# jalhajj/mahout

Measured on AMD Instinct MI355X. Metric: sketch updates/sec + item-pair cosines/sec @1M items, 1/2/4/8 MI355X, higher is better.
Workload: dtype u32

## Files before the change

mahout_amd/csrc/cms_build.hip:

```cpp
#include <hip/hip_runtime.h>

#include <algorithm>
#include <cstdlib>

#include "cms_device.h"
#include "cms_internal.h"

namespace cms {

#ifdef CMS_BUILD_CHEAPHASH
#define bucket(hp, d, kp) ((uint32_t)(((kp) >> (d)) & (hp).wmask))
#endif
#ifdef CMS_BUILD_GATHERHASH
#define bucket(hp, d, kp) \
  ((uint32_t)(((&(hp).gtab[(kp) & 0xFFFFFFu].x)[((d) >> 1) & 3] >> (((d) & 1) << 4)) & (hp).wmask))
#endif

struct HotInfo {
  int64_t row;
  int32_t nslices;
  int32_t e0;
};

constexpr int kKeyRegs = 4;

typedef unsigned short u16x2 __attribute__((ext_vector_type(2)));

__device__ __forceinline__ uint32_t nibbles8(uint32_t lo, uint32_t hi) {
  return __builtin_amdgcn_perm(hi | (hi >> 4), lo | (lo >> 4), 0x06040200u);
}

__global__ void k_build_plan(const int64_t* lo_, const int64_t* hi_, int64_t nrows, int64_t split, int64_t slice,
                             int first, int32_t* row_hot, HotInfo* hot, int2* extra_map,
                             uint32_t* counters , uint64_t* norm, uint32_t* rowmax,
                             int depth) {
  const int lane = (int)__lane_id();
  for (int64_t base = blockIdx.x * (int64_t)blockDim.x; base < nrows; base += (int64_t)gridDim.x * blockDim.x) {
    const int64_t r = base + threadIdx.x;
    const int64_t c = r < nrows ? hi_[r] - lo_[r] : 0;
    const bool is_hot = c > split;
    if (r < nrows && !is_hot) row_hot[r] = -1;
    int32_t ns = 0;
    uint32_t hidx = 0, e0 = 0;
    if (is_hot) {
      ns = (int32_t)((c + slice - 1) / slice);
      const unsigned long long old =
          atomicAdd(reinterpret_cast<unsigned long long*>(counters), ((unsigned long long)(ns - first) << 32) | 1ULL);
      hidx = (uint32_t)old;
      e0 = (uint32_t)(old >> 32);
      hot[hidx] = HotInfo{r, ns, (int32_t)e0};
      row_hot[r] = (int32_t)hidx;
      for (int d = 0; d < depth; ++d) norm[r * depth + d] = 0;
      rowmax[r] = 0;
    }
    unsigned long long m = __ballot(is_hot);
    while (m) {
      const int l = __builtin_ctzll(m);
      m &= m - 1;
      const int32_t nsl = __builtin_amdgcn_readlane(ns, l);
      const uint32_t hl = (uint32_t)__builtin_amdgcn_readlane((int)hidx, l);
      const uint32_t el = (uint32_t)__builtin_amdgcn_readlane((int)e0, l);
      for (int32_t sl = first + lane; sl < nsl; sl += 64) extra_map[el + sl - first] = make_int2((int)hl, sl);
    }
  }
}

__global__ void k_row_bound_implicit(const int64_t* lo_, const int64_t* hi_, int64_t nrows, int fb, int64_t slice, const uint64_t* old_mass,
                                     uint64_t* bound, uint8_t* force) {
  for (int64_t r = blockIdx.x * (int64_t)blockDim.x + threadIdx.x; r < nrows; r += (int64_t)gridDim.x * blockDim.x) {
    const int64_t c = hi_[r] - lo_[r];
    bound[r] = ((uint64_t)c << fb) + (old_mass ? old_mass[r] : 0ULL);
    force[r] = c > slice ? 1 : 0;
  }
}

__global__ __launch_bounds__(256) void k_row_bound_values(const int64_t* lo_, const int64_t* hi_, const float* vals, int64_t nrows, int fb,
                                                          int64_t slice, const uint64_t* old_mass, uint64_t* bound,
                                                          uint8_t* force) {
  __shared__ uint64_t red[4];
  for (int64_t r = blockIdx.x; r < nrows; r += gridDim.x) {
    uint64_t s = 0;
    for (int64_t i = lo_[r] + threadIdx.x; i < hi_[r]; i += 256) {
      uint32_t inc;
      if (load_inc(vals, i, inc, fb)) s += inc;
    }
    s = block_sum_u64_sat(s, red);
    if (threadIdx.x == 0) {
      bound[r] = sat_add(s, old_mass ? old_mass[r] : 0ULL);
      force[r] = (hi_[r] - lo_[r]) > slice ? 1 : 0;
    }
  }
}

constexpr int64_t kByteKeys = 64 * kKeyRegs;
__device__ __forceinline__ bool byte_class(int32_t slot, int64_t nkeys, uint64_t bound) {
  return slot < 0 && nkeys <= kByteKeys && bound < 256;
}

typedef uint32_t u32x4_t __attribute__((ext_vector_type(4)));
__device__ __forceinline__ void store_row(uint4* p, uint4 v, int sv) {
  if (sv == 2) {
    const u32x4_t x = {v.x, v.y, v.z, v.w};
    __builtin_nontemporal_store(x, reinterpret_cast<u32x4_t*>(p));
  } else {
    *p = v;
  }
}

#ifdef CMS_NO_SLICE_PAIRS
constexpr bool kNoSlicePairs = true;
#else
constexpr bool kNoSlicePairs = false;
#endif
constexpr int kBuildStoreForm = 2;
constexpr size_t kFormLdsMax = 64 * 1024;

constexpr int kBuildWaves = 6;
template <int SV>
__global__ __launch_bounds__(kBuildThreads) __attribute__((amdgpu_waves_per_eu(kBuildWaves, 8))) void k_build_rows(
    const int64_t* lo_, const int64_t* hi_, Keys keys, const float* vals, int64_t nrows, HashParams hp,
    int64_t slice,
    const int32_t* row_hot, const HotInfo* hot, const int2* extra_map, const uint32_t* counters, int64_t emax,
    TableView tv, uint64_t* row_mass, uint64_t* norm, uint32_t* rowmax, uint32_t* flags, int accumulate,
    int slices_done, const uint64_t* bound, int forms, int skip_untouched, int32_t* hidx_w, uint32_t* cbound,
    const int32_t* rows_list, const uint32_t* rows_cnt) {
  extern __shared__ __align__(16) uint32_t lds[];
  __shared__ unsigned long long s_norm[CMS_MAX_DEPTH];
  __shared__ unsigned long long s_mass;
  __shared__ uint32_t s_max;
  const int w = (int)hp.width;
  const int64_t dw = (int64_t)hp.depth * w;
  const int tid = threadIdx.x;

  int64_t row, lo, hi;
  bool atomic_mode;
  if (blockIdx.x < emax) {
    if (slices_done || blockIdx.x >= counters[1]) return;
#ifdef CMS_BUILD_NOSLICES
    return;
#endif
    int2 m = extra_map[blockIdx.x];
    row = hot[m.x].row;
    lo = lo_[row] + (int64_t)m.y * slice;
    hi = min(hi_[row], lo + slice);
    atomic_mode = true;
  } else {
    row = (int64_t)blockIdx.x - emax;
    if (rows_list) {
      if (row >= (int64_t)*rows_cnt) return;
      row = rows_list[row];
    }
    lo = lo_[row];
    atomic_mode = row_hot[row] >= 0;
    if (atomic_mode && slices_done) return;
    hi = atomic_mode ? lo + slice : hi_[row];
    if (skip_untouched && hi_[row] == lo) return;
// ... 472 lines not shown
            const int64_t i = base + tid + (int64_t)u * MTH;
            inc4[u] = 0;
            if (i < hi) {
              uint32_t inc;
              if (!load_inc(vals, i, inc, hp.frac_bits)) {
                badv = true;
                inc = 0;
              }
              inc4[u] = inc;
            }
          }
          if (base + kStep < hi) fetch(base + kStep);
#pragma unroll
          for (int u = 0; u < 4; ++u) {
            if (inc4[u]) add_all(keys.resolve(kk[u]), inc4[u], -1);
            mass += inc4[u];
          }
        }
        mass_pending = false;
      }
      if (__ballot(ovf) && (tid & 63) == 0) s_ovf = 1u;
      __syncthreads();
      const bool fits = s_ovf == 0u;
      __syncthreads();
      if (fits) level = 0;
      if (fits && tele) {
#pragma unroll
        for (int d = 0; d < kSq; ++d) {
          const uint32_t sq = wave_sum_u32(sqr[d]);
          if ((tid & 63) == 0 && sq) atomicAdd(&s_norm[d], (unsigned long long)sq);
        }
        level = 3;
      }
    }
    if (level == 3) level = 0;
    else if (level == 0) {
      const uint4* l4 = reinterpret_cast<const uint4*>(lds);
      const int nq = w >> 5;
      for (int d = 0; d < hp.depth; ++d) {
        uint32_t sq = 0;
        for (int j = tid; j < nq; j += MTH) {
          const uint4 v = l4[d * nq + j];
          const uint32_t x[4] = {v.x, v.y, v.z, v.w};
#pragma unroll
          for (int q = 0; q < 4; ++q) {
            const uint32_t lo4 = x[q] & 0x0F0F0F0Fu, hi4 = (x[q] >> 4) & 0x0F0F0F0Fu;
            sq = __builtin_amdgcn_udot4(lo4, lo4, sq, false);
            sq = __builtin_amdgcn_udot4(hi4, hi4, sq, false);
          }
#ifdef CMS_BUILD_NOWRITE
          if (false)
#endif
          if (!as_list) store_row(d4 + d * nq + j, v, SV);
        }
        sq = wave_sum_u32(sq);
        if ((tid & 63) == 0 && sq) atomicAdd(&s_norm[d], (unsigned long long)sq);
      }
    }
    if (level < 0) level = start > 1 ? 2 : 1;
    else level = -level - 1;
    for (;;) {
      if (level < 0) break;
      const int bits = 4 << level;
      const int lg = 3 - level;
      const uint32_t cap = (1u << bits) - 1u;
      const int nq = (w * bits) >> 7;
      uint4* l4 = reinterpret_cast<uint4*>(lds);
      if (tid < CMS_MAX_DEPTH) s_norm[tid] = 0ULL;
      if (tid == 0) {
        s_max = 0u;
        s_ovf = 0u;
        s_mass = 0ULL;
      }
      vmax = 0;
      for (int d = 0; d < hp.depth; ++d) {
        for (int j = tid; j < nq; j += MTH) l4[j] = make_uint4(0, 0, 0, 0);
        __syncthreads();
        uint64_t sq = 0;
        bool ovf = false;
        auto add = [&](uint64_t kr, uint32_t inc) {
          const uint32_t c = bucket(hp, d, kr);
          const uint32_t sh = (c & ((1u << lg) - 1u)) * (uint32_t)bits;
          const uint32_t old = (atomicAdd(&lds[c >> lg], inc << sh) >> sh) & cap;
          const uint32_t nv = old + inc;
          ovf |= nv > cap || inc > cap;
          sq += (uint64_t)(2u * old + inc) * inc;
          vmax = max(vmax, nv);
        };
        if (cached) {
#pragma unroll
          for (int k = 0; k < MKR; ++k)
            if (ik[k]) add(kp[k], ik[k]);
        } else {
          for (int64_t base = lo; base < hi; base += kMidRowKeys * MTH) {
            uint64_t kk[kMidRowKeys];
            uint32_t inc4[kMidRowKeys];
#pragma unroll
            for (int u = 0; u < kMidRowKeys; ++u) {
              const int64_t i = base + tid + (int64_t)u * MTH;
              kk[u] = i < hi ? keys.at(i) : 0;
              inc4[u] = 0;
              if (i < hi) {
                uint32_t inc;
                if (!load_inc(vals, i, inc, hp.frac_bits)) {
                  badv = true;
                  inc = 0;
                }
                inc4[u] = inc;
              }
            }
#pragma unroll
            for (int u = 0; u < kMidRowKeys; ++u) {
              if (inc4[u]) add(kk[u], inc4[u]);
              if (mass_pending) mass += inc4[u];
            }
          }
          mass_pending = false;
        }
        sq = wave_sum_u64_sat(sq);
        if ((tid & 63) == 0 && sq) atomicAdd(&s_norm[d], (unsigned long long)sq);
        if (__ballot(ovf) && (tid & 63) == 0) s_ovf = 1u;
        __syncthreads();
        if (s_ovf) break;
#ifdef CMS_BUILD_NOWRITE
        if (false)
#endif
        if (!(as_list && level == 1))
          for (int j = tid; j < nq; j += MTH) store_row(d4 + d * nq + j, l4[j], SV);
        __syncthreads();
      }
      if (!s_ovf || level == 2) break;
      __syncthreads();
      ++level;
    }
    if (level < 0) level = -level - 1;
    if (badv) atomicOr(flags, kFlagBadValue);
#pragma unroll
    for (int o = 32; o > 0; o >>= 1) vmax = max(vmax, (uint32_t)__shfl_xor((int)vmax, o, 64));
    if ((tid & 63) == 0 && vmax) atomicMax(&s_max, vmax);
    mass = wave_sum_u64_sat(mass);
    if ((tid & 63) == 0 && mass) atomicAdd(&s_mass, (unsigned long long)mass);
    __syncthreads();
    if (tid < hp.depth) norm[row * hp.depth + tid] = s_norm[tid];
    const bool listed = as_list && level <= 1;
    if (tid == 0) {
      rowmax[row] = s_max;
      row_mass[row] = s_mass;
      if (s_mass >= (1ULL << 32)) atomicOr(flags, kFlagOverflow);
      if (listed) lst[0] = (uint16_t)m;
      hidx_w[row] = listed ? kFormList : level == 0 ? kFormU4 : level == 1 ? kFormU8 : kFormU16;
      cbound[row] = s_max;
    }
    __syncthreads();
  }
}

constexpr int kStreamThreads = 512;
constexpr int kStreamPer = 2;
constexpr int kStreamRedWords = 1 + (kStreamThreads / 64) * (CMS_MAX_DEPTH + 2);
template <int SV, int D>
__device__ __forceinline__ void mid_streamed(const int64_t* lo_, const int64_t* hi_, const Keys& keys,
                                             const HashParams& hp, const int32_t* list, const uint32_t* list_cnt,
                                             uint32_t cap, const TableView& tv, int32_t* hidx_w, uint32_t* cbound,
                                             uint64_t* row_mass, uint64_t* norm, uint32_t* rowmax, int32_t* redo,
                                             uint32_t* redo_cnt, uint32_t* ticket, int u4_keys, int u8_keys) {
  extern __shared__ __align__(16) uint32_t lds[];
  constexpr int T = kStreamThreads;
  constexpr int NW = T / 64;
  constexpr int RS = CMS_MAX_DEPTH + 2;
  const int tid = threadIdx.x, lane = tid & 63, wv = tid >> 6;
  const int w = (int)hp.width;
  const int depth = D > 0 ? D : hp.depth;
  const int nq = w >> 4;
  const uint32_t nfront = list_cnt[0], count = nfront + list_cnt[1];
  uint4* l4 = reinterpret_cast<uint4*>(lds);
  uint32_t* red = lds + 1;
  if (tid == 0) lds[0] = atomicAdd(ticket, 1u);
  __syncthreads();
  uint32_t li = lds[0];
  while (li < count) {
    __syncthreads();
    const int64_t row = list2_at(list, cap, nfront, li);
    const int64_t lo = lo_[row], hi = hi_[row];
    const int64_t m = hi - lo;
    const bool u8_start = m > u4_keys && m <= u8_keys;
    uint32_t mine = 0;
    uint32_t bytes = 0;
    u16x2 pm = {0, 0};
    if (u8_start) {
      for (int j = tid; j < depth * nq; j += T) l4[j] = make_uint4(0, 0, 0, 0);
      __syncthreads();
      constexpr int64_t kStep = (int64_t)kStreamPer * T;
      uint64_t nx[kStreamPer];
      auto fetch = [&](int64_t base) {
#pragma unroll
        for (int u = 0; u < kStreamPer; ++u) {
          const int64_t i = base + tid + (int64_t)u * T;
          nx[u] = i < hi ? keys.raw(i) : 0ULL;
        }
      };
      fetch(lo);
      for (int64_t base = lo; base < hi; base += kStep) {
        uint64_t kk[kStreamPer];
#pragma unroll
        for (int u = 0; u < kStreamPer; ++u) kk[u] = nx[u];
        if (base + kStep < hi) fetch(base + kStep);
#pragma unroll
        for (int u = 0; u < kStreamPer; ++u) {
          if (base + tid + (int64_t)u * T >= hi) continue;
          each_bucket<D>(hp, keys.resolve(kk[u]), [&](int r, uint32_t bk) {
            const uint32_t c = (uint32_t)r * (uint32_t)w + bk;
            atomicAdd(&lds[c >> 2], 1u << ((c & 3u) << 3));
          });
        }
      }
      __syncthreads();
      uint4* d4 = reinterpret_cast<uint4*>(tv.row16(row));
      auto sweep_row = [&](int r) {
        uint32_t sq = 0;
        for (int j = tid; j < nq; j += T) {
          const uint4 v = l4[r * nq + j];
          const uint32_t x[4] = {v.x, v.y, v.z, v.w};
#pragma unroll
          for (int q = 0; q < 4; ++q) {
            sq = __builtin_amdgcn_udot4(x[q], x[q], sq, false);
            bytes = __builtin_amdgcn_udot4(x[q], 0x01010101u, bytes, false);
            pm = __builtin_elementwise_max(pm, __builtin_elementwise_max(__builtin_bit_cast(u16x2, x[q] & 0x00FF00FFu),
                                                                         __builtin_bit_cast(u16x2, (x[q] >> 8) & 0x00FF00FFu)));
          }
          store_row(d4 + r * nq + j, v, SV);
        }
        sq = wave_sum_u32(sq);
        if (lane == r) mine = sq;
      };
#pragma unroll 1
      for (int r = 0; r < depth; ++r) sweep_row(r);
    }
    uint32_t vmax = max((uint32_t)pm.x, (uint32_t)pm.y);
#pragma unroll
    for (int o = 32; o > 0; o >>= 1) vmax = max(vmax, (uint32_t)__shfl_xor((int)vmax, o, 64));
    bytes = wave_sum_u32(bytes);
    __syncthreads();
    if (lane < depth) red[wv * RS + lane] = mine;
    if (lane == 0) {
      red[wv * RS + CMS_MAX_DEPTH] = vmax;
      red[wv * RS + CMS_MAX_DEPTH + 1] = bytes;
    }
    if (tid == 0) lds[0] = atomicAdd(ticket, 1u);
    __syncthreads();
    uint32_t mx = 0, total = 0;
#pragma unroll
    for (int k = 0; k < NW; ++k) {
      mx = max(mx, red[k * RS + CMS_MAX_DEPTH]);
      total += red[k * RS + CMS_MAX_DEPTH + 1];
    }
    if (!u8_start || total != (uint32_t)depth * (uint32_t)m) {
      if (tid == 0) redo[atomicAdd(redo_cnt, 1u)] = (int32_t)row;
    } else {
      if (tid < depth) {
        uint64_t s = 0;
#pragma unroll
        for (int k = 0; k < NW; ++k) s += red[k * RS + tid];
        norm[row * depth + tid] = s;
      }
      if (tid == 0) {
        rowmax[row] = mx;
        row_mass[row] = (uint64_t)m;
        hidx_w[row] = kFormU8;
        cbound[row] = mx;
      }
    }
    li = lds[0];
  }
}

template <int SV, int D, int MT>
__global__ __launch_bounds__(MT) __attribute__((amdgpu_waves_per_eu(MT == kStreamThreads ? 8 : 4, 8))) void k_build_mid(
    const int64_t* lo_, const int64_t* hi_, Keys keys, const float* vals, HashParams hp,
    const int32_t* list, const uint32_t* list_cnt , uint32_t cap, TableView tv, int32_t* hidx_w,
    uint32_t* cbound, uint64_t* row_mass, uint64_t* norm, uint32_t* rowmax, uint32_t* flags, int list_keys,
    int u4_keys, int u8_keys, int32_t* redo, uint32_t* redo_cnt, uint32_t* ticket) {
  if constexpr (MT == kStreamThreads)
    mid_streamed<SV, D>(lo_, hi_, keys, hp, list, list_cnt, cap, tv, hidx_w, cbound, row_mass, norm, rowmax, redo,
                        redo_cnt, ticket, u4_keys, u8_keys);
  else
    mid_rows<SV, D, MT>(lo_, hi_, keys, vals, hp, list, list_cnt, cap, tv, hidx_w, cbound, row_mass, norm, rowmax,
                        flags, list_keys, u4_keys, u8_keys);
}

constexpr int kMidGridPerCu = 8;
constexpr int kNibWaves = 4;

__global__ void k_row_caps(const int64_t* lo_, const int64_t* hi_, int64_t n, const uint64_t* bound,
                           const int32_t* hidx, int forms, int weighted, int frac_bits, int d, int w, int bit_keys,
                           int crumb_keys, int list_keys, uint32_t* caps) {
  const int64_t dw = (int64_t)d * w;
  const uint32_t full = (uint32_t)(slot_units(dw) / kRowAlign);
  for (int64_t r = blockIdx.x * (int64_t)blockDim.x + threadIdx.x; r < n; r += (int64_t)gridDim.x * blockDim.x) {
    const int32_t s = hidx[r];
    const int64_t m = hi_[r] - lo_[r];
    uint32_t c = full;
    if (s >= 0) {
      c = 0;
    } else if (forms && byte_class(s, m, bound[r])) {
      const int64_t u16s = nib_list_row(m, w, d, weighted != 0, frac_bits, bit_keys, crumb_keys, list_keys)
                               ? 1 + (int64_t)d * m
                               : dw / 2;
      c = (uint32_t)((u16s + kRowAlign - 1) / kRowAlign);
    }
    caps[r] = c;
  }
}

template <int SV>
__device__ __forceinline__ void nib_owner(
    int64_t row, uint32_t* lds, const int64_t* lo_, const int64_t* hi_, const Keys& keys, const float* vals,
    const HashParams& hp, const int32_t* row_hot, const uint64_t* bound, const TableView& tv, int32_t* hidx_w,
    uint32_t* cbound, uint64_t* row_mass, uint64_t* norm, uint32_t* rowmax, uint32_t* flags, int32_t* redo,
    uint32_t* redo_cnt, int bit_keys, int crumb_keys, int list_keys, int lists_done) {
  const int lane = threadIdx.x & 63;
  const int wv = threadIdx.x >> 6;
  const int64_t lo = lo_[row], hi = hi_[row];
  if (row_hot[row] >= 0 || !byte_class(tv.hidx[row], hi - lo, bound[row])) return;
  const int w = (int)hp.width;
  if (lists_done && nib_list_row(hi - lo, w, hp.depth, vals != nullptr, hp.frac_bits, bit_keys, crumb_keys, list_keys))
    return;
  uint64_t kp[kKeyRegs];
  uint32_t ik[kKeyRegs];
  uint32_t mass = 0;
  bool badv = false;
#pragma unroll
  for (int k = 0; k < kKeyRegs; ++k) {
    const int64_t i = lo + lane + (int64_t)k * 64;
    kp[k] = 0;
    ik[k] = 0;
    if (i < hi) {
      uint32_t inc;
      if (!load_inc(vals, i, inc, hp.frac_bits)) {
        badv = true;
        inc = 0;
      }
      kp[k] = keys.at(i);
      ik[k] = inc;
      mass += inc;
    }
  }
  const int64_t m = hi - lo;
  int bits = nib_first_bits(m, w, bit_keys, crumb_keys);
  const bool as_list = nib_list_row(m, w, hp.depth, vals != nullptr, hp.frac_bits, bit_keys, crumb_keys, list_keys);
  if (as_list) bits = 4;
  uint16_t* lst = tv.row16(row);
  uint4* slot4 = reinterpret_cast<uint4*>(lds) + wv * (w >> 5);
  uint32_t* slot = lds + wv * (w >> 3);
  uint4* d4 = reinterpret_cast<uint4*>(tv.row16(row));
  uint32_t vmax = 0;
  bool ovf = false;
  for (;;) {
    const int lg = bits == 1 ? 5 : bits == 2 ? 4 : 3;
    const uint32_t cap = (1u << bits) - 1u;
    const int nq = (w * bits) >> 7;
    vmax = 0;
    ovf = false;
    for (int d = 0; d < hp.depth; ++d) {
      for (int j = lane; j < nq; j += 64) slot4[j] = make_uint4(0, 0, 0, 0);
      uint32_t sq = 0;
#pragma unroll
      for (int k = 0; k < kKeyRegs; ++k)
        if (ik[k]) {
// ... 376 lines not shown
#pragma unroll
    for (int r = 0; r < D; ++r) sq[r] = 0u;
    uint32_t vmax = 0;
    const int nf = min(max((m - lane + 63) >> 6, 0), NSL);
    const uint32_t live = (1u << nf) - 1u;
    const int ns = (m + 63) >> 6;
    const bool ovf = mid_list_rows<D>(slot, pk, live, ns, sq, vmax);
    if (ovf) {
      if (lane == 0) redo[atomicAdd(redo_cnt, 1u)] = row;
    } else {
#pragma unroll
      for (int r = 0; r < D; ++r) sq[r] = wave_fold_dpp(sq[r], [](uint32_t a, uint32_t b) { return a + b; });
      vmax = wave_fold_dpp(vmax, [](uint32_t a, uint32_t b) { return max(a, b); });
      if (lane < D) {
        uint32_t s = 0;
#pragma unroll
        for (int r = 0; r < D; ++r)
          if (lane == r) s = sq[r];
        norm[(int64_t)row * D + lane] = s;
      }
      if (lane == 0) {
        lst[0] = (uint16_t)m;
        rowmax[row] = vmax;
        row_mass[row] = (uint64_t)m;
        hidx_w[row] = kFormList;
        cbound[row] = vmax;
      }
    }
    if (row1 < 0) break;
    row = row1;
    lo = nlo;
    m = nm;
    base = nbase;
    raw0 = nraw0;
    row1 = row2;
  }
}

template <int SV>
__global__ __launch_bounds__(kBuildThreads) void k_build_bytes(
    const int64_t* lo_, const int64_t* hi_, Keys keys, const float* vals, HashParams hp,
    const int32_t* list, const uint32_t* list_cnt, TableView tv, int32_t* hidx_w, uint32_t* cbound,
    uint64_t* row_mass, uint64_t* norm, uint32_t* rowmax, uint32_t* flags) {
  extern __shared__ __align__(16) uint32_t lds[];
  __shared__ unsigned long long s_norm[CMS_MAX_DEPTH];
  __shared__ uint32_t s_max, s_mass;
  const int tid = threadIdx.x;
  const int w = (int)hp.width;
  const int64_t dw = (int64_t)hp.depth * w;
  const uint32_t count = *list_cnt;
  for (uint32_t li = blockIdx.x; li < count; li += gridDim.x) {
    const bool keep_list = list[li] < 0;
    const int64_t row = keep_list ? ~(int64_t)list[li] : (int64_t)list[li];
    const int64_t lo = lo_[row], hi = hi_[row];
    uint16_t* lst = tv.row16(row);
    if (tid < CMS_MAX_DEPTH) s_norm[tid] = 0ULL;
    if (tid == 0) {
      s_max = 0u;
      s_mass = 0u;
    }
    uint64_t kp[kKeyRegs];
    uint32_t ik[kKeyRegs];
    uint32_t mass = 0;
    bool badv = false;
#pragma unroll
    for (int k = 0; k < kKeyRegs; ++k) {
      const int64_t i = lo + tid + (int64_t)k * kBuildThreads;
      kp[k] = 0;
      ik[k] = 0;
      if (i < hi) {
        uint32_t inc;
        if (!load_inc(vals, i, inc, hp.frac_bits)) {
          badv = true;
          inc = 0;
        }
        kp[k] = keys.at(i);
        ik[k] = inc;
        mass += inc;
      }
    }
    const int nq = (int)(dw >> 4);
    uint4* l4 = reinterpret_cast<uint4*>(lds);
    for (int j = tid; j < nq; j += kBuildThreads) l4[j] = make_uint4(0, 0, 0, 0);
    __syncthreads();
    uint32_t vmax = 0;
    for (int d = 0; d < hp.depth; ++d) {
      uint32_t sq = 0;
#pragma unroll
      for (int k = 0; k < kKeyRegs; ++k)
        if (ik[k]) {
          const uint32_t bk = bucket(hp, d, kp[k]);
          const uint32_t c = (uint32_t)d * (uint32_t)w + bk;
          if (keep_list) lst[1 + (int64_t)d * (hi - lo) + tid + (int64_t)k * kBuildThreads] = (uint16_t)bk;
          const uint32_t sh = (c & 3u) << 3;
          const uint32_t old = (atomicAdd(&lds[c >> 2], ik[k] << sh) >> sh) & 255u;
          sq += (2u * old + ik[k]) * ik[k];
          vmax = max(vmax, old + ik[k]);
        }
      sq = wave_sum_u32(sq);
      if ((tid & 63) == 0 && sq) atomicAdd(&s_norm[d], (unsigned long long)sq);
    }
#pragma unroll
    for (int o = 32; o > 0; o >>= 1) vmax = max(vmax, (uint32_t)__shfl_xor((int)vmax, o, 64));
    if ((tid & 63) == 0 && vmax) atomicMax(&s_max, vmax);
    mass = wave_sum_u32(mass);
    if ((tid & 63) == 0 && mass) atomicAdd(&s_mass, mass);
    __syncthreads();
    uint4* d4 = reinterpret_cast<uint4*>(lst);
#ifdef CMS_BUILD_NOWRITE
    if (false)
#endif
    if (!keep_list)
      for (int j = tid; j < nq; j += kBuildThreads) store_row(d4 + j, l4[j], SV);
    if (badv) atomicOr(flags, kFlagBadValue);
    if (tid < hp.depth) norm[row * hp.depth + tid] = s_norm[tid];
    if (tid == 0) {
      rowmax[row] = s_max;
      row_mass[row] = s_mass;
      hidx_w[row] = keep_list ? kFormList : kFormU8;
      cbound[row] = s_max;
    }
    __syncthreads();
  }
}

constexpr int kSliceThreads = 512;
constexpr bool kWholeSlices = true;
constexpr int64_t kHotSlice = 65535;
template <int D>
__global__ __launch_bounds__(kSliceThreads) void k_build_slices(const int64_t* lo_, const int64_t* hi_, Keys keys,
                                                                HashParams hp, int64_t slice, const HotInfo* hot,
                                                                const int2* smap, const uint32_t* counters,
                                                                TableView tv, uint64_t* row_mass, uint32_t* flags,
                                                                int whole, uint64_t* norm, uint32_t* rowmax) {
  extern __shared__ __align__(16) uint32_t lds[];
  const uint32_t nsl = counters[1];
  if (blockIdx.x >= nsl) return;
  const int tid = threadIdx.x;
  const uint32_t stride = (nsl % 7919u) ? 7919u : 7907u;
  const uint32_t sidx = (uint32_t)(((uint64_t)blockIdx.x * stride) % nsl);
  const int2 m = smap[sidx];
  const int64_t row = hot[m.x].row;
  const int64_t lo = lo_[row] + (int64_t)m.y * slice;
  const int64_t end = min(hi_[row], lo + slice);
  const int w = (int)hp.width;
  const int64_t dw = (int64_t)hp.depth * w;
  const int words = (int)(dw >> 1);
  uint4* l4 = reinterpret_cast<uint4*>(lds);
  for (int j = tid; j < (words >> 2); j += kSliceThreads) l4[j] = make_uint4(0, 0, 0, 0);
  for (int j = (words & ~3) + tid; j < words; j += kSliceThreads) lds[j] = 0u;
  __syncthreads();
  const uint32_t one = 1u << hp.frac_bits;
  constexpr int kPer = 8;
  constexpr int64_t kStep = kPer * kSliceThreads;
  uint64_t nx[kPer];
  auto fetch = [&](int64_t base) {
#pragma unroll
    for (int u = 0; u < kPer; ++u) {
      const int64_t i = base + tid + (int64_t)u * kSliceThreads;
      nx[u] = i < end ? keys.raw(i) : 0ULL;
    }
  };
  if (lo < end) fetch(lo);
  for (int64_t base = lo; base < end; base += kStep) {
    uint64_t kk[kPer];
#pragma unroll
    for (int u = 0; u < kPer; ++u) kk[u] = nx[u];
    if (base + kStep < end) fetch(base + kStep);
#pragma unroll
    for (int u = 0; u < kPer; ++u) {
      if (base + tid + (int64_t)u * kSliceThreads >= end) continue;
      const uint64_t kp = keys.resolve(kk[u]);
      each_bucket<D>(hp, kp, [&](int r, uint32_t bk) {
        const uint32_t c = (uint32_t)r * (uint32_t)w + bk;
#ifdef CMS_BUILD_NOLDSADD
        if (c == 0xFFFFFFFFu)
#endif
        atomicAdd(&lds[c >> 1], one << ((c & 1u) << 4));
      });
    }
  }
  __syncthreads();
  if (whole && hot[m.x].nslices == 1) {
    u32x4_t* o4 = reinterpret_cast<u32x4_t*>(tv.hot + (int64_t)tv.hidx[row] * dw);
    const uint2* s2 = reinterpret_cast<const uint2*>(lds);
    uint32_t vmax = 0;
    for (int r = 0; r < hp.depth; ++r) {
      uint64_t sq = 0;
      const int q0 = r * (w >> 2), q1 = q0 + (w >> 2);
      for (int q = q0 + tid; q < q1; q += kSliceThreads) {
        const uint2 v = s2[q];
        const uint32_t c0 = v.x & 0xFFFFu, c1 = v.x >> 16, c2 = v.y & 0xFFFFu, c3 = v.y >> 16;
        sq += (uint64_t)c0 * c0 + (uint64_t)c1 * c1 + (uint64_t)c2 * c2 + (uint64_t)c3 * c3;
        vmax = max(max(vmax, max(c0, c1)), max(c2, c3));
        const u32x4_t x = {c0, c1, c2, c3};
        __builtin_nontemporal_store(x, o4 + q);
      }
      sq = wave_sum_u64_sat(sq);
      if ((tid & 63) == 0 && sq) atomicAdd((unsigned long long*)&norm[row * hp.depth + r], (unsigned long long)sq);
    }
#pragma unroll
    for (int o = 32; o > 0; o >>= 1) vmax = max(vmax, (uint32_t)__shfl_xor((int)vmax, o, 64));
    if ((tid & 63) == 0 && vmax) atomicMax(&rowmax[row], vmax);
  } else {
    unsigned long long* dst = reinterpret_cast<unsigned long long*>(tv.hot + (int64_t)tv.hidx[row] * dw);
    const int units = (words + 63) >> 6;
    const int rot = (int)(((uint32_t)m.y * 2654435761u >> 8) % (uint32_t)units) << 6;
    for (int jj = tid; jj < words; jj += kSliceThreads) {
      const int j = jj + rot < words ? jj + rot : jj + rot - words;
      const uint32_t v = lds[j];
#ifdef CMS_BUILD_NOSLICEADD
      if (v == 0xFFFFFFFFu)
#endif
      if (v) atomicAdd(dst + j, (unsigned long long)(v & 0xFFFFu) | ((unsigned long long)(v >> 16) << 32));
    }
  }
  if (tid == 0) {
    const uint64_t tm = (uint64_t)(end - lo) * one;
    const unsigned long long old = atomicAdd((unsigned long long*)&row_mass[row], (unsigned long long)tm);
    if (old + tm >= (1ULL << 32)) atomicOr(flags, kFlagOverflow);
  }
}

__global__ __launch_bounds__(256) void k_hot_norms(const HotInfo* hot, const uint32_t* counters, HashParams hp,
                                                   TableView tv, uint64_t* norm, uint32_t* rowmax, int whole_slices) {
  __shared__ uint64_t red[4];
  const uint32_t nhot = counters[0];
  const int d = blockIdx.y;
  const int w = (int)hp.width;
  for (uint32_t hb = blockIdx.x; hb < nhot; hb += gridDim.x) {
    if (hot[hb].nslices <= whole_slices) continue;
    const int64_t row = hot[hb].row;
    const uint32_t* p = tv.hot + (int64_t)tv.hidx[row] * tv.dw + (int64_t)d * w;
    uint64_t sq = 0;
    uint32_t vmax = 0;
    if ((w & 3) == 0 && (((uintptr_t)p) & 15) == 0) {
      const uint4* p4 = reinterpret_cast<const uint4*>(p);
      for (int j = threadIdx.x; j < (w >> 2); j += 256) {
        const uint4 v = p4[j];
        sq = sat_add(sq, (uint64_t)v.x * v.x + (uint64_t)v.y * v.y);
        sq = sat_add(sq, (uint64_t)v.z * v.z + (uint64_t)v.w * v.w);
        vmax = max(vmax, max(max(v.x, v.y), max(v.z, v.w)));
      }
    } else {
      for (int j = threadIdx.x; j < w; j += 256) {
        sq = sat_add(sq, (uint64_t)p[j] * p[j]);
        vmax = max(vmax, p[j]);
      }
    }
#pragma unroll
    for (int o = 32; o > 0; o >>= 1) vmax = max(vmax, (uint32_t)__shfl_xor((int)vmax, o, 64));
    if ((threadIdx.x & 63) == 0 && vmax) atomicMax(&rowmax[row], vmax);
    uint64_t tot = block_sum_u64_sat(sq, red);
    if (tot > (1ULL << 60)) tot = 1ULL << 60;
    if (threadIdx.x == 0) atomicAdd((unsigned long long*)&norm[row * hp.depth + d], (unsigned long long)tot);
  }
}

int row_bounds(cms_handle* h, const int64_t* d_lo, const int64_t* d_hi, const float* d_val, const uint64_t* old_mass,
               int64_t slice, uint64_t* bound, uint8_t* force) {
  const int64_t n = h->n;
  if (d_val)
    hipLaunchKernelGGL(k_row_bound_values, dim3((unsigned)std::max<int64_t>(1, std::min<int64_t>(n, 65536))),
                       dim3(256), 0, h->stream, d_lo, d_hi, d_val, n, h->hp.frac_bits, slice, old_mass, bound, force);
  else
    hipLaunchKernelGGL(k_row_bound_implicit, dim3((unsigned)std::max<int64_t>(1, std::min<int64_t>((n + 255) / 256, 4096))),
                       dim3(256), 0, h->stream, d_lo, d_hi, n, h->hp.frac_bits, slice, old_mass, bound, force);
  CMS_HIP(hipGetLastError());
  return CMS_OK;
}

int ingest_csr_device(cms_handle* h, const int64_t* d_off, const int64_t* d_key, const float* d_val, int64_t npairs) {
  h->rf_valid = false;
  return ingest_spans_device(h, d_off, d_off + 1, d_key, nullptr, d_val, npairs);
}

int ingest_spans_device(cms_handle* h, const int64_t* d_lo, const int64_t* d_hi, const int64_t* d_key,
                        const uint32_t* d_tok, const float* d_val, int64_t npairs) {
  const Keys keys{d_key, d_tok};
  const int64_t n = h->n;
  int rc0;
  const int accumulate = h->empty ? 0 : 1;
  int64_t kSplit = cms::kSlice;
  if (h->p.width >= 8192) kSplit *= 2;
  if (h->tune.split_keys > 0) kSplit = h->tune.split_keys;
  const size_t img_lds = (size_t)h->dw * 2;
  const bool fast_slices = !d_val && (h->dw % 8) == 0 && img_lds <= 80 * 1024 && h->hp.frac_bits < 16;
  const int64_t kSliceKeys = fast_slices ? (kHotSlice >> h->hp.frac_bits) : kSplit;
  const int whole_slices =
      kWholeSlices && fast_slices && !accumulate && (h->p.width % 4) == 0 ? 1 : 0;
  const int64_t max_hot = std::min<int64_t>(n, npairs / kSplit + 1);
  const int64_t emax = npairs / kSliceKeys + max_hot + 1;
  const size_t sz_rowhot = (sizeof(int32_t) * (size_t)n + 15) & ~size_t(15);
  const size_t sz_hot = (sizeof(HotInfo) * (size_t)max_hot + 15) & ~size_t(15);
  const size_t sz_extra = sizeof(int2) * (size_t)emax;
  CMS_HIP(h->ws_hot.ensure(sz_rowhot + sz_hot + sz_extra + 64));
  char* base = h->ws_hot.as<char>();
  int32_t* row_hot = reinterpret_cast<int32_t*>(base);
  HotInfo* hot = reinterpret_cast<HotInfo*>(base + sz_rowhot);
  int2* extra_map = reinterpret_cast<int2*>(base + sz_rowhot + sz_hot);
  uint32_t* counters = h->d_flags + 4;
  struct PlanSide {
    cms_handle* h;
    bool on = false;
    void end() {
      if (!on) return;
      on = false;
      std::swap(h->stream, h->side_stream);
      h->plan_side_active = false;
      if (hipEventRecord(h->ev_plan, h->side_stream) == hipSuccess) (void)hipStreamWaitEvent(h->stream, h->ev_plan, 0);
    }
    ~PlanSide() { end(); }
  } plan_side{h};
  if (h->spans_event && !accumulate && !d_val && h->side_stream) {
    h->spans_event = false;
    CMS_HIP(hipStreamWaitEvent(h->side_stream, h->ev_spans, 0));
    std::swap(h->stream, h->side_stream);
    h->plan_side_active = true;
    plan_side.on = true;
  }
  CMS_HIP(hipMemsetAsync(counters, 0, 4 * sizeof(uint32_t), h->stream));
  {
    TimedScope ts(h, "build_plan");
    if (!accumulate && (rc0 = reset_table_layout(h))) return rc0;
    DevBuf& bound = h->ws_bound;
    DevBuf& force = h->ws_force;
    CMS_HIP(bound.ensure(sizeof(uint64_t) * (size_t)std::max<int64_t>(n, 1)));
    CMS_HIP(force.ensure((size_t)std::max<int64_t>(n, 1)));
    if ((rc0 = row_bounds(h, d_lo, d_hi, d_val, accumulate ? h->d_row_mass : nullptr, kSplit, bound.as<uint64_t>(),
                          force.as<uint8_t>())))
      return rc0;
    int64_t max_new = -1;
    if (!accumulate && !d_val && h->hp.frac_bits < 16) {
// ... 230 lines not shown
```

mahout_amd/csrc/cms_hash.h:

```cpp
#pragma once
#include <math.h>
#include <stdint.h>

#ifndef CMS_HD
#define CMS_HD __host__ __device__ __forceinline__
#endif

#define CMS_MAX_DEPTH 32

namespace cms {

constexpr uint64_t kPrime = 9223372036854775783ULL;
constexpr uint64_t kMask63 = 0x7FFFFFFFFFFFFFFFULL;

struct HashParams {
  uint64_t ap[CMS_MAX_DEPTH];
  uint64_t bp[CMS_MAX_DEPTH];
  uint64_t barrett;
  uint32_t width;
  uint32_t wmask;
  int32_t depth;
  int32_t pow2;
  int32_t frac_bits;
  int32_t fastq;
  double qa[CMS_MAX_DEPTH];
  double qb[CMS_MAX_DEPTH];
#ifdef CMS_BUILD_GATHERHASH
  const uint4* gtab;
#endif
};

inline void hash_finish(HashParams& hp) {
  hp.pow2 = hp.width != 0 && (hp.width & (hp.width - 1)) == 0;
  hp.wmask = hp.pow2 ? hp.width - 1u : 0u;
  hp.barrett = hp.pow2 ? 0 : (~0ULL) / (uint64_t)hp.width;
  hp.fastq = hp.pow2 && hp.width <= (1u << 24);
  for (int i = 0; i < CMS_MAX_DEPTH; ++i) {
    hp.qa[i] = i < hp.depth ? (double)((long double)hp.ap[i] / (long double)kPrime) : 0.0;
    hp.qb[i] = i < hp.depth ? (double)((long double)hp.bp[i] / (long double)kPrime) : 0.0;
  }
}

CMS_HD uint64_t reduce_key(int64_t k) {
  const int64_t P = (int64_t)kPrime;
  if (k >= 0) return (uint64_t)(k >= P ? k - P : k);
  int64_t t = k + P;
  if (t < 0) t += P;
  return (uint64_t)t;
}

CMS_HD uint64_t mulmod_p(uint64_t x, uint64_t y) {
  unsigned __int128 prod = (unsigned __int128)x * y;
  uint64_t lo = (uint64_t)prod;
  uint64_t hi = (uint64_t)(prod >> 64);
  uint64_t H = (hi << 1) | (lo >> 63);
  uint64_t L = lo & kMask63;
  unsigned __int128 t = (unsigned __int128)H * 25u;
  uint64_t tH = (uint64_t)(t >> 63);
  uint64_t tL = (uint64_t)t & kMask63;
  uint64_t z = tL + L;
  if (z >= kPrime) z -= kPrime;
  if (z >= kPrime) z -= kPrime;
  z += tH * 25u;
  if (z >= kPrime) z -= kPrime;
  return z;
}

CMS_HD uint64_t mulmod_p_small(uint64_t x, uint32_t y) {
  const uint64_t p0 = (uint64_t)(uint32_t)x * y;
  const uint64_t p1 = (x >> 32) * (uint64_t)y;
  const uint64_t lo = p0 + (p1 << 32);
  const uint64_t hi = (p1 >> 32) + (lo < p0 ? 1u : 0u);
  const uint64_t H = (hi << 1) | (lo >> 63);
  uint64_t z = (lo & kMask63) + H * 25u;
  if (z >= kPrime) z -= kPrime;
  return z;
}

CMS_HD uint32_t bucket_exact(const HashParams& hp, int r, uint64_t kp) {
  uint64_t s = ((kp >> 32) == 0 ? mulmod_p_small(hp.ap[r], (uint32_t)kp) : mulmod_p(hp.ap[r], kp)) + hp.bp[r];
  if (s >= kPrime) s -= kPrime;
  if (hp.pow2) return (uint32_t)(s & hp.wmask);
  uint64_t q = (uint64_t)(((unsigned __int128)s * hp.barrett) >> 64);
  uint64_t rem = s - q * hp.width;
  while (rem >= hp.width) rem -= hp.width;
  return (uint32_t)rem;
}

#if defined(__HIP_DEVICE_COMPILE__)
#define CMS_MUL24(x, y) __umul24((x), (y))
#else
#define CMS_MUL24(x, y) (((x) & 0xFFFFFFu) * ((y) & 0xFFFFFFu))
#endif
constexpr double kQEps = 1.0 / 65536.0;

CMS_HD uint32_t bucket_q(const HashParams& hp, int r, uint64_t kp, double kf, uint32_t km) {
  const double y = fma(hp.qa[r], kf, hp.qb[r]);
  const double fl = floor(y);
  const double fr = y - fl;
  union {
    double d;
    uint64_t u;
  } qb;
  qb.d = fl + 4503599627370496.0;
  uint32_t q = (uint32_t)qb.u;
  if (!(fr >= kQEps && fr <= 1.0 - kQEps)) {
    const uint64_t q0 = qb.u & 0xFFFFFFFFFFFFFULL;
    const uint64_t x = hp.ap[r] * kp + hp.bp[r];
    const uint64_t s = x - ((q0 << 63) - 25u * q0);
    if (s >= kPrime) q = fr < 0.5 ? q - 1u : q + 1u;
  }
  const uint32_t xm = CMS_MUL24((uint32_t)hp.ap[r] & hp.wmask, km) + (uint32_t)hp.bp[r];
  return (xm + CMS_MUL24(q, 25u)) & hp.wmask;
}

CMS_HD uint32_t bucket(const HashParams& hp, int r, uint64_t kp) {
  if (hp.fastq && (kp >> 32) == 0) return bucket_q(hp, r, kp, (double)(uint32_t)kp, (uint32_t)kp & hp.wmask);
  return bucket_exact(hp, r, kp);
}

template <int D, typename F>
CMS_HD void each_bucket(const HashParams& hp, uint64_t kp, F&& f) {
#ifdef CMS_BUILD_CHEAPHASH
  if (D > 0) {
#pragma unroll
    for (int r = 0; r < D; ++r) f(r, (uint32_t)((kp >> r) & hp.wmask));
  } else {
    for (int r = 0; r < hp.depth; ++r) f(r, (uint32_t)((kp >> r) & hp.wmask));
  }
  return;
#endif
#ifdef CMS_BUILD_GATHERHASH
  {
    const uint4 e = hp.gtab[kp & 0xFFFFFFu];
    const uint32_t v[4] = {e.x, e.y, e.z, e.w};
    for (int r = 0; r < (D > 0 ? D : hp.depth); ++r) f(r, (v[(r >> 1) & 3] >> ((r & 1) << 4)) & hp.wmask);
    return;
  }
#endif
  if (D > 0) {
    if (hp.fastq && (kp >> 32) == 0) {
      const double kf = (double)(uint32_t)kp;
      const uint32_t km = (uint32_t)kp & hp.wmask;
#pragma unroll
      for (int r = 0; r < D; ++r) f(r, bucket_q(hp, r, kp, kf, km));
    } else {
#pragma unroll
      for (int r = 0; r < D; ++r) f(r, bucket_exact(hp, r, kp));
    }
  } else {
    for (int r = 0; r < hp.depth; ++r) f(r, bucket(hp, r, kp));
  }
}

CMS_HD uint32_t bucket_wb(const HashParams& hp, int r, uint64_t kp, uint32_t w, uint64_t barrett) {
  uint64_t s = mulmod_p(hp.ap[r], kp) + hp.bp[r];
  if (s >= kPrime) s -= kPrime;
  uint64_t q = (uint64_t)(((unsigned __int128)s * barrett) >> 64);
  uint64_t rem = s - q * w;
  while (rem >= w) rem -= w;
  return (uint32_t)rem;
}

CMS_HD uint64_t residue_wbq(const HashParams& hp, int r, uint64_t kp) {
  if ((kp >> 32) != 0) {
    uint64_t s = mulmod_p(hp.ap[r], kp) + hp.bp[r];
    if (s >= kPrime) s -= kPrime;
    return s;
  }
  const double y = fma(hp.qa[r], (double)(uint32_t)kp, hp.qb[r]);
  const double fl = floor(y);
  const double fr = y - fl;
  union {
    double d;
    uint64_t u;
  } qb;
  qb.d = fl + 4503599627370496.0;
  const uint64_t q = qb.u & 0xFFFFFFFFFFFFFULL;
  uint64_t s = hp.ap[r] * kp + hp.bp[r] - ((q << 63) - 25u * q);
  if (s >= kPrime) s = fr < 0.5 ? s + kPrime : s - kPrime;
  return s;
}

CMS_HD uint32_t mod_barrett(uint64_t s, uint32_t w, uint64_t barrett) {
  const uint64_t qq = (uint64_t)(((unsigned __int128)s * barrett) >> 64);
  uint64_t rem = s - qq * w;
  while (rem >= w) rem -= w;
  return (uint32_t)rem;
}

CMS_HD uint32_t bucket_wbq(const HashParams& hp, int r, uint64_t kp, uint32_t w, uint64_t barrett) {
  return mod_barrett(residue_wbq(hp, r, kp), w, barrett);
}

}
```

Baseline: 55.59 billion.

## Add row-hash fast path with deferred exact redo for streamed and sliced sketch builds

Introduces a RowHash struct that caches per-row hash coefficients in registers and computes all depth buckets with a single min/max check on the fractional part. Keys near a rounding boundary are flagged and recomputed exactly in a separate redo pass, so the common path avoids per-row branching. A shared key_pass helper replaces the duplicated prefetch loops, and the slice kernel reads 32-bit tokens directly when available instead of 64-bit raw keys. This reduces hash ALU work and divergence, at the cost of more register pressure and a second loop for rare keys.

```diff
diff --git a/mahout_amd/csrc/cms_build.hip b/mahout_amd/csrc/cms_build.hip
--- a/mahout_amd/csrc/cms_build.hip
+++ b/mahout_amd/csrc/cms_build.hip
@@ -2,6 +2,7 @@
 
 #include <algorithm>
 #include <cstdlib>
+#include <type_traits>
 
 #include "cms_device.h"
 #include "cms_internal.h"
@@ -780,6 +781,54 @@
       cbound[row] = s_max;
     }
     __syncthreads();
+  }
+}
+
+#if defined(CMS_BUILD_CHEAPHASH) || defined(CMS_BUILD_GATHERHASH)
+constexpr bool kRowHash = false;
+#else
+constexpr bool kRowHash = true;
+#endif
+
+struct NoRedo {};
+template <typename R, int PER, int T, typename L, typename F, typename G>
+__device__ __forceinline__ void key_pass(int64_t lo, int64_t end, int tid, L&& load, F&& f, G&& g) {
+  constexpr int64_t kStep = (int64_t)PER * T;
+  R nx[PER];
+  auto fetch = [&](int64_t base) {
+#pragma unroll
+    for (int u = 0; u < PER; ++u) {
+      const int64_t i = base + tid + (int64_t)u * T;
+      nx[u] = i < end ? load(i) : R(0);
+    }
+  };
+  if (lo < end) fetch(lo);
+  for (int64_t base = lo; base < end; base += kStep) {
+    R kk[PER];
+#pragma unroll
+    for (int u = 0; u < PER; ++u) kk[u] = nx[u];
+    if (base + kStep < end) fetch(base + kStep);
+    const int live = (int)min(end - base, kStep);
+    if constexpr (std::is_same<typename std::decay<G>::type, NoRedo>::value) {
+#pragma unroll
+      for (int u = 0; u < PER; ++u)
+        if (tid < live - u * T) f(kk[u]);
+    } else {
+      uint32_t left = 0;
+#pragma unroll
+      for (int u = 0; u < PER; ++u)
+        if (tid < live - u * T && f(kk[u])) left |= 1u << u;
+      if (left) {
+#pragma unroll 1
+        for (int u = 0; u < PER; ++u) {
+          if (!((left >> u) & 1u)) continue;
+          R k = kk[0];
+#pragma unroll
+          for (int j = 1; j < PER; ++j) k = j == u ? kk[j] : k;
+          g(k);
+        }
+      }
+    }
   }
 }
 
@@ -818,30 +867,41 @@
     if (u8_start) {
       for (int j = tid; j < depth * nq; j += T) l4[j] = make_uint4(0, 0, 0, 0);
       __syncthreads();
-      constexpr int64_t kStep = (int64_t)kStreamPer * T;
-      uint64_t nx[kStreamPer];
-      auto fetch = [&](int64_t base) {
-#pragma unroll
-        for (int u = 0; u < kStreamPer; ++u) {
-          const int64_t i = base + tid + (int64_t)u * T;
-          nx[u] = i < hi ? keys.raw(i) : 0ULL;
-        }
+      auto add = [&](int r, uint32_t bk) {
+        const uint32_t c = (uint32_t)r * (uint32_t)w + bk;
+        atomicAdd(&lds[c >> 2], 1u << ((c & 3u) << 3));
       };
-      fetch(lo);
-      for (int64_t base = lo; base < hi; base += kStep) {
-        uint64_t kk[kStreamPer];
-#pragma unroll
-        for (int u = 0; u < kStreamPer; ++u) kk[u] = nx[u];
-        if (base + kStep < hi) fetch(base + kStep);
-#pragma unroll
-        for (int u = 0; u < kStreamPer; ++u) {
-          if (base + tid + (int64_t)u * T >= hi) continue;
-          each_bucket<D>(hp, keys.resolve(kk[u]), [&](int r, uint32_t bk) {
-            const uint32_t c = (uint32_t)r * (uint32_t)w + bk;
-            atomicAdd(&lds[c >> 2], 1u << ((c & 3u) << 3));
-          });
-        }
-      }
+      constexpr int DR = D > 0 ? D : 1;
+      const RowHash<DR> rh(hp);
+      const bool fast = kRowHash && D > 0 && hp.fastq, tok = keys.tok != nullptr;
+      key_pass<uint64_t, kStreamPer, T>(
+          lo, hi, tid, [&](int64_t i) { return keys.raw(i); },
+          [&](uint64_t raw) {
+            if (!fast) {
+              each_bucket<(kRowHash ? 0 : D)>(hp, keys.resolve(raw), add);
+              return false;
+            }
+            uint32_t bk[DR];
+            uint32_t k = (uint32_t)raw;
+            bool again = k >= kTokEscape;
+            if (!tok) {
+              const uint64_t kp = reduce_key((int64_t)raw);
+              k = (uint32_t)kp;
+              again = kp >= kRowHashKeyEnd;
+            }
+            if (rh.rows32(k, bk) || again) {
+              const uint64_t kp = keys.resolve(raw);
+#pragma unroll 1
+              for (int r = 0; r < D; ++r) add(r, bucket(hp, r, kp));
+              return false;
+            }
+#pragma unroll
+            for (int r = 0; r < D; ++r)
+              atomicAdd(reinterpret_cast<uint32_t*>(reinterpret_cast<char*>(lds) + ((uint32_t)r * (uint32_t)w + (bk[r] & ~3u))),
+                        1u << ((bk[r] << 3) & 31u));
+            return false;
+          },
+          NoRedo{});
       __syncthreads();
       uint4* d4 = reinterpret_cast<uint4*>(tv.row16(row));
       auto sweep_row = [&](int r) {
@@ -1524,33 +1584,63 @@
   __syncthreads();
   const uint32_t one = 1u << hp.frac_bits;
   constexpr int kPer = 8;
-  constexpr int64_t kStep = kPer * kSliceThreads;
-  uint64_t nx[kPer];
-  auto fetch = [&](int64_t base) {
-#pragma unroll
-    for (int u = 0; u < kPer; ++u) {
-      const int64_t i = base + tid + (int64_t)u * kSliceThreads;
-      nx[u] = i < end ? keys.raw(i) : 0ULL;
-    }
+  auto add = [&](int r, uint32_t bk) {
+    const uint32_t c = (uint32_t)r * (uint32_t)w + bk;
+#ifdef CMS_BUILD_NOLDSADD
+    if (c == 0xFFFFFFFFu)
+#endif
+    atomicAdd(&lds[c >> 1], one << ((c & 1u) << 4));
   };
-  if (lo < end) fetch(lo);
-  for (int64_t base = lo; base < end; base += kStep) {
-    uint64_t kk[kPer];
-#pragma unroll
-    for (int u = 0; u < kPer; ++u) kk[u] = nx[u];
-    if (base + kStep < end) fetch(base + kStep);
-#pragma unroll
-    for (int u = 0; u < kPer; ++u) {
-      if (base + tid + (int64_t)u * kSliceThreads >= end) continue;
-      const uint64_t kp = keys.resolve(kk[u]);
-      each_bucket<D>(hp, kp, [&](int r, uint32_t bk) {
-        const uint32_t c = (uint32_t)r * (uint32_t)w + bk;
+  if (kRowHash && D > 0 && hp.fastq) {
+    constexpr int DR = D > 0 ? D : 1;
+    RowHash<DR> rh(hp);
+    rh.vgpr();
+    const uint32_t w2 = 2u * (uint32_t)w;
+    auto add_rows = [&](const uint32_t (&bk)[DR]) {
+#pragma unroll
+      for (int r = 0; r < D; ++r) {
+        uint32_t* p = reinterpret_cast<uint32_t*>(reinterpret_cast<char*>(lds) + ((uint32_t)r * w2 | ((bk[r] << 1) & ~3u)));
 #ifdef CMS_BUILD_NOLDSADD
-        if (c == 0xFFFFFFFFu)
+        if (bk[r] == 0xFFFFFFFFu)
 #endif
-        atomicAdd(&lds[c >> 1], one << ((c & 1u) << 4));
-      });
-    }
+        atomicAdd(p, one << ((bk[r] << 4) & 31u));
+      }
+    };
+    auto redo_key = [&](uint64_t kp) {
+#pragma unroll 1
+      for (int r = 0; r < D; ++r) add(r, bucket(hp, r, kp));
+    };
+    if (keys.tok) {
+      const uint32_t* tok = keys.tok;
+      key_pass<uint32_t, kPer, kSliceThreads>(
+          lo, end, tid, [&](int64_t i) { return tok[i]; },
+          [&](uint32_t t) {
+            uint32_t bk[DR];
+            if (rh.rows32(t, bk) || t >= kTokEscape) return true;
+            add_rows(bk);
+            return false;
+          },
+          [&](uint32_t t) { redo_key(keys.resolve(t)); });
+    } else {
+      const int64_t* key = keys.key;
+      key_pass<int64_t, kPer, kSliceThreads>(
+          lo, end, tid, [&](int64_t i) { return key[i]; },
+          [&](int64_t k) {
+            uint32_t bk[DR];
+            if (rh.rows(reduce_key(k), bk)) return true;
+            add_rows(bk);
+            return false;
+          },
+          [&](int64_t k) { redo_key(reduce_key(k)); });
+    }
+  } else {
+    key_pass<uint64_t, kPer, kSliceThreads>(
+        lo, end, tid, [&](int64_t i) { return keys.raw(i); },
+        [&](uint64_t raw) {
+          each_bucket<D>(hp, keys.resolve(raw), add);
+          return false;
+        },
+        NoRedo{});
   }
   __syncthreads();
   if (whole && hot[m.x].nslices == 1) {
diff --git a/mahout_amd/csrc/cms_hash.h b/mahout_amd/csrc/cms_hash.h
--- a/mahout_amd/csrc/cms_hash.h
+++ b/mahout_amd/csrc/cms_hash.h
@@ -153,6 +153,59 @@
   }
 }
 
+constexpr uint32_t kFracHiMin = 0x3EF00000u;
+constexpr uint32_t kFracHiMax = 0x3FEFFFDFu;
+constexpr uint64_t kRowHashKeyEnd = 0xFFFFFFFEULL;
+template <int D>
+struct RowHash {
+  double qa[D], qb[D];
+  uint32_t am[D], bm[D];
+  uint32_t wmask;
+  CMS_HD explicit RowHash(const HashParams& hp) : wmask(hp.wmask) {
+#pragma unroll
+    for (int r = 0; r < D; ++r) {
+      qa[r] = hp.qa[r];
+      qb[r] = hp.qb[r];
+      am[r] = (uint32_t)hp.ap[r] & hp.wmask;
+      bm[r] = (uint32_t)hp.bp[r];
+    }
+  }
+  CMS_HD void vgpr() {
+#if defined(__HIP_DEVICE_COMPILE__)
+#pragma unroll
+    for (int r = 0; r < D; ++r) {
+      asm volatile("" : "+v"(qb[r]));
+      asm volatile("" : "+v"(bm[r]));
+    }
+#endif
+  }
+  CMS_HD bool rows32(uint32_t k, uint32_t (&bk)[D]) const {
+    const double kf = (double)k;
+    const uint32_t km = k & wmask;
+    uint32_t lo = 0xFFFFFFFFu, hi = 0u;
+#pragma unroll
+    for (int r = 0; r < D; ++r) {
+      const double y = fma(qa[r], kf, qb[r]);
+#if defined(__HIP_DEVICE_COMPILE__)
+      const double fr = __builtin_amdgcn_fract(y);
+      const uint32_t q = (uint32_t)y;
+#else
+      const double fr = y - floor(y);
+      const uint32_t q = (uint32_t)(int64_t)y;
+#endif
+      const uint32_t fh = (uint32_t)(__builtin_bit_cast(uint64_t, fr) >> 32);
+      lo = fh < lo ? fh : lo;
+      hi = fh > hi ? fh : hi;
+      bk[r] = (CMS_MUL24(am[r], km) + bm[r] + CMS_MUL24(q, 25u)) & wmask;
+    }
+    return lo < kFracHiMin || hi > kFracHiMax;
+  }
+  CMS_HD bool rows(uint64_t kp, uint32_t (&bk)[D]) const {
+    const bool far = kp >= kRowHashKeyEnd;
+    return rows32((uint32_t)kp, bk) || far;
+  }
+};
+
 CMS_HD uint32_t bucket_wb(const HashParams& hp, int r, uint64_t kp, uint32_t w, uint64_t barrett) {
   uint64_t s = mulmod_p(hp.ap[r], kp) + hp.bp[r];
   if (s >= kPrime) s -= kPrime;
```

Measured after the change: 59.57 billion (median of 6 runs). 7.2% higher.
